# cheolwanpark/tiny-raytracer

Measured on AMD Instinct MI355X. Metric: Mray/s (primary+secondary), higher is better.
Workload: dtype f32; 1 GPU; cornell 2048x2048, depth 50, 256 spp per step (of 4096), streamed, reference-order BVH, seed 1; rays=160658711950, samples=22548578304, image_rows_per_gpu=2048, tuning=default, parallelism=single GPU, world_size=1, launched_by=plain

## Files before the change

### tiny-raytracer_amd/csrc/capi.hip

```cpp
#include <hip/hip_runtime.h>

#include <math.h>
#include <stdio.h>
#include <stdlib.h>
#include <string.h>

#include <algorithm>
#include <memory>
#include <mutex>
#include <new>
#include <string>
#include <thread>
#include <vector>

#include "axis_quads.h"
#include "nearest_first.h"
#include "flat_reuse.h"
#include "host_stage.h"
#include "kernels.h"
#include "scene.h"
#include "scene_adopt.h"
#include "scene_cache.h"
#include "scene_query.h"
#include "stream_plan.h"
// ... 29 lines not shown
        if (hipEventCreate(&ev) != hipSuccess) { (void)hipGetLastError(); return; }
        if (hipEventRecord(ev, stream) != hipSuccess) { (void)hipGetLastError(); (void)hipEventDestroy(ev); return; }
        t_open.ev = ev; t_open.stream = stream; t_open.device = dev; t_open.epoch = epoch;
        return;
    }
    if (!t_open.ev) return;
    TimingOpen o = t_open;
    t_open = TimingOpen{};
    hipEvent_t ev = nullptr;
    if (o.stream != stream || o.device != dev || o.epoch != epoch || hipEventCreate(&ev) != hipSuccess) {
        (void)hipGetLastError();
        (void)hipEventDestroy(o.ev);
        return;
    }
    if (hipEventRecord(ev, stream) != hipSuccess) { (void)hipGetLastError(); (void)hipEventDestroy(ev); (void)hipEventDestroy(o.ev); return; }
    std::lock_guard<std::mutex> lock(g_timing_mu);
    if (g_timing_on && g_timing_epoch == epoch) g_timing_pairs.push_back(TimingPair{o.ev, ev, dev});
    else { (void)hipEventDestroy(o.ev); (void)hipEventDestroy(ev); }
}
}

struct trt_scene {
    SceneHost host;
    FlatReuse flat_reuse{};
    std::vector<uint32_t> geo_index;
    SceneCache cache;
};

namespace {

thread_local std::string g_last_error;

int fail(int code, const std::string& msg) {
    g_last_error = msg;
    return code;
}
int fail_hip(hipError_t e, const char* what) {
    return fail(TRT_ERR_HIP, std::string(what) + ": " + hipGetErrorString(e));
}
#define TRT_HIP(call)                                        \
    do {                                                     \
        hipError_t e_ = (call);                              \
        if (e_ != hipSuccess) return fail_hip(e_, #call);    \
    } while (0)

struct Defaults {
    trt_tuning tuning;
    trt_scene_options scene;
    bool flat_reuse = true;
    bool axis_quads = true;
    bool nearest_first = true;
    uint32_t flat_literal = 2;
    bool flat_literal_test_fail = false;
};
const Defaults& defaults() {
    static const Defaults d = [] {
        Defaults x;
        x.tuning = tuning_builtin();
        x.scene = scene_options_builtin();
        auto env = [](const char* name) -> const char* { const char* e = getenv(name); return (e && *e) ? e : nullptr; };
        auto u32 = [&](const char* name, uint32_t& field) { if (const char* e = env(name)) field = (uint32_t)strtoul(e, nullptr, 10); };
        trt_tuning& t = x.tuning;
        u32("TRT_STREAM_MINW", t.stream_waves_per_simd); u32("TRT_BIG_THREADS", t.stream_big_threads); u32("TRT_STREAM_BATCH_SPP", t.stream_batch_spp);
        u32("TRT_RADIANCE_GB", t.radiance_gb); u32("TRT_LEAF_SLOTS", t.leaf_slots); u32("TRT_LDS_LEAF_STACK", t.lds_leaf_stack);
        u32("TRT_RAY_POOL", t.ray_pool); u32("TRT_STRAGGLERS", t.stragglers); u32("TRT_LDS_STRAGGLERS", t.lds_stragglers);
        u32("TRT_DUAL_WALK", t.dual_walk); u32("TRT_RUNTIME_WALK", t.runtime_walk); u32("TRT_XCD_REMAP", t.xcd_remap);
        u32("TRT_MINW", t.mega_waves_per_simd); u32("TRT_MEGA_THREADS", t.mega_threads); u32("TRT_MINW8", t.mega_global_waves8);
        u32("TRT_WF_MINW", t.wf_waves_per_simd); u32("TRT_WF_SERVE_MIN", t.wf_serve_min);
        trt_scene_options& o = x.scene;
        if (const char* e = env("TRT_CULL_PRUNE")) {
            const float v = (float)atof(e);
            if (v > 0.0f && v <= 1.0f) o.cull_prune = v;
        }
        if (const char* e = env("TRT_FLAT_WALK")) o.flat_walk = atoi(e) ? 1 : 0;
        if (const char* e = env("TRT_FLAT_REUSE")) x.flat_reuse = atoi(e) != 0;
        if (const char* e = env("TRT_AXIS_QUADS")) x.axis_quads = atoi(e) != 0;
        if (const char* e = env("TRT_NEAREST_FIRST")) x.nearest_first = atoi(e) != 0;
        if (const char* e = env("TRT_FLAT_LITERAL")) x.flat_literal = atoi(e) != 0 ? 1u : 0u;
        if (const char* e = env("TRT_FLAT_LITERAL_TEST_FAIL")) x.flat_literal_test_fail = atoi(e) != 0;
        if (const char* e = env("TRT_COMPACT_NODES")) o.compact_nodes = atoi(e) ? 1 : 0;
        if (const char* e = env("TRT_SCRATCH_CAP_MB")) o.scratch_cap_bytes = (uint64_t)strtoull(e, nullptr, 10) << 20;
        return x;
    }();
    return d;
}

[[maybe_unused]] const bool g_defaults_read_at_load = (defaults(), true);

int require_device() {
    int n = 0;
    hipError_t e = hipGetDeviceCount(&n);
    if (e != hipSuccess || n <= 0) {
        (void)hipGetLastError();
        return fail(TRT_ERR_NO_DEVICE, "no HIP device visible: libtinyrt has no CPU path, it needs a gfx950 GPU");
    }
    return TRT_OK;
}

int scene_on_device(trt_scene* s, SceneDev& out) {
    out.L = s->host.layout;
    return s->cache.on_device(SceneCache::PACKED_SCENE, s->host.blob.data(), s->host.layout.blob_bytes, "scene upload", out.blob);
}

void to_camera_dev(const trt_camera& c, CameraDev& d) {
    const trt_vec3* src[6] = {&c.position, &c.viewport_upper_left, &c.horizontal, &c.vertical, &c.defocus_disk_u, &c.defocus_disk_v};
    float* dst[6] = {d.pos, d.upper_left, d.horizontal, d.vertical, d.du, d.dv};
    for (int i = 0; i < 6; i++) { dst[i][0] = src[i]->x; dst[i][1] = src[i]->y; dst[i][2] = src[i]->z; }
    d.width = c.width;
    d.height = c.height;
}

int to_render_args(const trt_camera* cam, const trt_render_params* p, RenderArgs& ra, uint32_t& rows, trt_tuning& tn) {
    if (cam->width < 2 || cam->height < 2) return fail(TRT_ERR_INVALID_ARG, "camera width and height must be at least 2 (pointgen.rs:41-42 divides by width-1, height-1)");
    if (p->samples_per_pixel == 0) return fail(TRT_ERR_INVALID_ARG, "samples_per_pixel must be positive");
    uint32_t s1 = p->sample_end == 0 ? p->samples_per_pixel : p->sample_end;
    if (p->sample_begin > s1 || s1 > p->samples_per_pixel) return fail(TRT_ERR_INVALID_ARG, "sample range must satisfy begin <= end <= samples_per_pixel");
    if (p->backend > TRT_BACKEND_STREAMED) return fail(TRT_ERR_INVALID_ARG, "unknown backend");
    ra.background[0] = p->background.x; ra.background[1] = p->background.y; ra.background[2] = p->background.z;
    ra.inv_spp = 1.0f / (float)p->samples_per_pixel;
    ra.max_bounces = p->max_bounces;
    ra.seed_key = rng_seed_key(p->seed);
    ra.sample_begin = p->sample_begin;
    ra.sample_end = s1;
    ra.accumulate = p->accumulate ? 1u : 0u;
    if (p->band_rows == 0) {
        ra.band_rows = 0; ra.band_stride = 1; ra.band_offset = 0;
        rows = cam->height;
    } else {
        if (p->band_stride == 0 || p->band_offset >= p->band_stride) return fail(TRT_ERR_INVALID_ARG, "band_offset must be below band_stride");
        rows = p->rows_local;
        if (rows > 0) {
            uint32_t last = rows - 1;
// ... 39 lines not shown
    ra.flat_reuse = s->flat_reuse;
    const size_t bytes = (size_t)rows * cam->width * 3 * sizeof(float);
    if (rows == 0 || ra.sample_begin == ra.sample_end || ra.max_bounces == 0) {
        if (!ra.accumulate && bytes) TRT_HIP(hipMemsetAsync(d_accum, 0, bytes, stream));
        if (!ra.accumulate && bytes && d_moment2) TRT_HIP(hipMemsetAsync(d_moment2, 0, bytes, stream));
        return TRT_OK;
    }
    const bool wavefront = p->backend == TRT_BACKEND_WAVEFRONT;
    const bool streamed = p->backend == TRT_BACKEND_STREAMED || p->backend == TRT_BACKEND_AUTO;
    if (wavefront || streamed) {
        int dev = 0;
        TRT_HIP(hipGetDevice(&dev));
        Workspace* ws = nullptr;
        if (wavefront) {
            rc = s->cache.workspace_acquire(dev, wavefront_workspace_bytes(cam->width, rows), stream, &ws);
        } else {
            uint32_t samples = ra.sample_end - ra.sample_begin;
            const uint32_t full = streamed_chunk_spp(cam->width, rows, tn.radiance_gb);
            if (samples > full) samples = full;
            const uint32_t wanted = samples;
            const uint32_t short_samples = s->cache.short_samples(dev);
            if (short_samples != 0u && short_samples < samples) {
                const size_t idle = s->cache.idle_workspace_bytes(dev);
                size_t free_b = 0, total_b = 0;
                const bool known = hipMemGetInfo(&free_b, &total_b) == hipSuccess;
                (void)hipGetLastError();
                if (!known || free_b + idle < streamed_workspace_bytes(cam->width, rows, samples, tn.radiance_gb)) samples = short_samples;
            }
            bool trimmed = false;
            for (;;) {
                rc = s->cache.workspace_acquire(dev, streamed_workspace_bytes(cam->width, rows, samples, tn.radiance_gb), stream, &ws);
                if (rc != TRT_ERR_OOM) break;
                if (!trimmed) {
                    trimmed = true;
                    s->cache.trim(dev, 0);
                    continue;
                }
                if (samples <= 1u) break;
                samples = (samples + 1u) / 2u;
            }
            s->cache.set_short_samples(dev, (rc == TRT_OK && samples < wanted) ? samples : 0u);
        }
        if (rc != TRT_OK) return rc;
        LiteralRequest lit;
        const SceneLayout& L = s->host.layout;
        if (streamed && defaults().flat_literal != 0u && L.flat_walk != 0u && L.n_leaves > 0u &&
            s->host.blob.size() >= 16u * ((size_t)L.off_leaf_list + 2u * (size_t)L.n_leaves)) {
            lit.slot = s->cache.literal_kernel(dev);
            lit.leaf_list = s->host.blob.data() + 16u * (size_t)L.off_leaf_list;
            lit.n_leaves = L.n_leaves;
            const uint64_t call_samples = (uint64_t)cam->width * rows * (ra.sample_end - ra.sample_begin);
            lit.wanted = defaults().flat_literal == 1u || call_samples >= kLiteralAutoSamples;
            lit.empty_source = defaults().flat_literal_test_fail;
        }
        const LiteralScope lit_scope(lit.slot ? &lit : nullptr);
        hipError_t le;
        if (streamed && d_moment2) {
            le = launch_moments ? launch_moments(sc, cd, ra, tn, ws->ptr, ws->bytes, d_accum, d_moment2, reinterpret_cast<unsigned long long*>(d_counters),
                                                 p->collect_stats != 0, stream)
                                : hipErrorInvalidDeviceFunction;
        } else if (streamed) {
            le = launch_streamed(sc, cd, ra, tn, ws->ptr, ws->bytes, d_accum, reinterpret_cast<unsigned long long*>(d_counters), p->collect_stats != 0, stream);
        } else {
            le = launch_wavefront(sc, cd, ra, tn, ws->ptr, d_accum, reinterpret_cast<unsigned long long*>(d_counters), p->collect_stats != 0, stream);
        }
        rc = s->cache.workspace_release(dev, ws, stream);
        if (le != hipSuccess) return fail_hip(le, streamed ? "launch_streamed" : "launch_wavefront");
        return rc;
    }
    TRT_HIP(launch_megakernel(sc, cd, ra, tn, d_accum, reinterpret_cast<unsigned long long*>(d_counters), p->collect_stats != 0, stream));
    return TRT_OK;
}

void set_flat_reuse(trt_scene* s) {
    const SceneLayout& L = s->host.layout;
    const size_t end = 16u * ((size_t)L.off_leaf_list + 2u * (size_t)L.n_leaves);
    const bool have = L.flat_walk != 0u && L.n_leaves > 0u && s->host.blob.size() >= end;
    uint32_t m[3];
    flat_reuse_masks(have ? s->host.blob.data() + 16u * (size_t)L.off_leaf_list : nullptr, L.n_leaves, have && defaults().flat_reuse, m);
    const size_t qend = 16u * ((size_t)L.off_quad + 5u * (size_t)L.n_quads);
    const bool have_quads = have && L.n_quads > 0u && s->host.blob.size() >= qend;
    const uint32_t aq = axis_quads_flag(have_quads ? s->host.blob.data() + 16u * (size_t)L.off_quad : nullptr, L.n_quads, L.n_leaves, L.flat_walk != 0u,
                                        scene_mode(L) == 1, defaults().axis_quads);
    float planes[3];
    const uint32_t nf = nearest_first_flag(have ? s->host.blob.data() + 16u * (size_t)L.off_leaf_list : nullptr, L.n_leaves,
                                           have_quads ? s->host.blob.data() + 16u * (size_t)L.off_quad : nullptr, L.n_quads, L.n_spheres, aq,
                                           defaults().nearest_first, planes);
    s->flat_reuse = FlatReuse{m[0], m[1], m[2], aq, nf, planes[0], planes[1], planes[2]};
}

void set_geo_index(trt_scene* s) {
    const SceneLayout& L = s->host.layout;
    const std::vector<int32_t>& geo = s->host.reference.prim_geo;
    s->geo_index.assign((size_t)L.n_spheres + L.n_quads, 0xFFFFFFFFu);
    const size_t end = 16u * ((size_t)L.off_ref_nodes + 2u * (size_t)L.n_nodes);
    if (geo.size() < L.n_nodes || s->host.blob.size() < end) return;
    for (uint32_t i = 0; i < L.n_nodes; i++) {
        if (geo[i] < 0) continue;
        uint32_t link;
        memcpy(&link, s->host.blob.data() + 16u * ((size_t)L.off_ref_nodes + 2u * (size_t)i + 1u) + 12u, 4);
        const size_t slot = (size_t)(link & PRIM_INDEX_MASK) + ((link & PRIM_QUAD_BIT) ? L.n_spheres : 0u);
        if (!(link & NODE_INNER_BIT) && slot < s->geo_index.size()) s->geo_index[slot] = (uint32_t)geo[i];
    }
}

trt_scene* scene_from_host(SceneHost&& host, const trt_scene_options& opt) {
// ... 652 lines not shown
```

### tiny-raytracer_amd/csrc/flat_literal.h

```cpp
#pragma once

#include <stdint.h>
#include <stdio.h>
#include <string.h>

#include <string>

#include "flat_reuse.h"

namespace trt {

constexpr uint32_t kFlatLiteralMaxLeaves = 32u;

namespace flat_literal_detail {

inline void hex(std::string& s, uint32_t bits) {
    char b[16];
    snprintf(b, sizeof b, "0x%08x", bits);
    s += b;
}

inline void box(std::string& s, const uint32_t w[8], uint32_t axes) {
    static const char* const o[3] = {"%[ox]", "%[oy]", "%[oz]"};
    static const char* const inv[3] = {"%[ix]", "%[iy]", "%[iz]"};
// ... 31 lines not shown
inline bool flat_literal_asm(const void* leaf_list, uint32_t n_leaves, const uint32_t masks[3], std::string& out) {
    using namespace flat_literal_detail;
    if (leaf_list == nullptr || n_leaves == 0u || n_leaves > kFlatLiteralMaxLeaves) return false;
    const unsigned char* p = static_cast<const unsigned char*>(leaf_list);
    const uint32_t n = n_leaves;
    auto leaf = [&](uint32_t k, uint32_t w[8]) { memcpy(w, p + 32u * (size_t)k, 32u); };
    auto axes_of = [&](uint32_t k) {
        const uint32_t b = 1u << k;
        return k == 0u ? 7u : (((masks[0] & b) ? 0u : 1u) | ((masks[1] & b) ? 0u : 2u) | ((masks[2] & b) ? 0u : 4u));
    };
    std::string s;
    uint32_t w[8];
    s += "s_cmp_lg_u32 %[i], 0\n";
    s += "s_cbranch_scc1 900f\n";
    for (uint32_t k = 0; k < n; k++) {
        label(s, 200u, k);
        leaf(k, w);
        box(s, w, axes_of(k));
        if ((k & 1u) && k + 1u < n) {
            s += "v_cmp_gt_u32_e32 vcc, %[top], %[lim]\n";
            s += "s_cbranch_vccnz "; ref(s, 400u, k + 1u, 'f'); s += "\n";
        }
    }
    s += "s_mov_b32 %[i], "; hex(s, n); s += "\n";
    s += "s_branch 990f\n";
    for (uint32_t k = 2; k < n; k += 2u) {
        label(s, 400u, k);
        s += "s_mov_b32 %[i], "; hex(s, k); s += "\n";
        s += "s_branch 990f\n";
    }
    for (uint32_t k = 2; k < n; k += 2u) {
        if (axes_of(k) == 7u) continue;
        label(s, 100u, k);
        leaf(k, w);
        box(s, w, 7u);
        if (k + 1u < n) { s += "s_branch "; ref(s, 200u, k + 1u, 'b'); s += "\n"; }
        else { s += "s_mov_b32 %[i], "; hex(s, n); s += "\n"; s += "s_branch 990f\n"; }
    }
    s += "900:\n";
    s += "s_lshl_b32 s38, %[i], 1\n";
    s += "s_add_u32 s38, s38, 12\n";
    s += "s_getpc_b64 s[36:37]\n";
    s += "s_add_u32 s36, s36, s38\n";
    s += "s_addc_u32 s37, s37, 0\n";
    s += "s_setpc_b64 s[36:37]\n";
    for (uint32_t k = 0; k < n; k += 2u) {
        s += "s_branch "; ref(s, axes_of(k) == 7u ? 200u : 100u, k, 'b'); s += "\n";
    }
    s += "990:\n";
    out.swap(s);
    return true;
}

inline std::string flat_literal_define(const std::string& name, const std::string& asm_text) {
    std::string d = "#define " + name + " \\\n";
    size_t a = 0;
    while (a < asm_text.size()) {
        size_t b = asm_text.find('\n', a);
        if (b == std::string::npos) b = asm_text.size();
        d += "\""; d.append(asm_text, a, b - a); d += "\\n\" \\\n";
        a = b + 1u;
    }
    d += "\"\"\n";
    return d;
}

}
```

### tiny-raytracer_amd/csrc/flat_literal_rtc.h

```cpp
#pragma once

#include <dlfcn.h>
#include <stdint.h>

#include <string>
#include <vector>

#include "flat_literal.h"

namespace trt {

struct RtcHeader { const char* name; const char* text; };
inline const std::vector<RtcHeader>& rtc_project_headers() {
    static const std::vector<RtcHeader> h = {
#include "rtc_headers.inc"
    };
    return h;
}
inline const std::vector<RtcHeader>& rtc_system_headers() {
    static const std::vector<RtcHeader> h = {
        {"hip/hip_runtime.h", "#pragma once\n"},
        {"stdint.h", "#pragma once\n"
                     "typedef signed char int8_t; typedef unsigned char uint8_t; typedef short int16_t; typedef unsigned short uint16_t;\n"
                     "typedef int int32_t; typedef unsigned int uint32_t; typedef long int64_t; typedef unsigned long uint64_t;\n"
                     "typedef unsigned long uintptr_t; typedef long intptr_t;\n"},
        {"stddef.h", "#pragma once\n#ifndef offsetof\n#define offsetof(t, m) __builtin_offsetof(t, m)\n#endif\n"},
        {"string.h", "#pragma once\ninline void* memcpy(void* d, const void* s, unsigned long n) { return __builtin_memcpy(d, s, n); }\n"},
        {"math.h", "#pragma once\n"},
    };
    return h;
}

struct HiprtcApi {
    typedef void* Program;
    int (*create)(Program*, const char*, const char*, int, const char* const*, const char* const*) = nullptr;
    int (*destroy)(Program*) = nullptr;
    int (*add_name)(Program, const char*) = nullptr;
    int (*compile)(Program, int, const char* const*) = nullptr;
    int (*log_size)(Program, size_t*) = nullptr;
    int (*log)(Program, char*) = nullptr;
    int (*lowered)(Program, const char*, const char**) = nullptr;
    int (*code_size)(Program, size_t*) = nullptr;
    int (*code)(Program, char*) = nullptr;
    bool ok = false;
};
inline const HiprtcApi& hiprtc_api(const void* beside) {
    static const HiprtcApi api = [beside] {
        HiprtcApi a;
        void* h = nullptr;
        for (const char* name : {"libhiprtc.so", "libhiprtc.so.7", "libhiprtc.so.6"}) {
            h = dlopen(name, RTLD_NOW | RTLD_LOCAL);
            if (h) break;
        }
        Dl_info info;
        if (!h && beside && dladdr(beside, &info) && info.dli_fname) {
            std::string dir(info.dli_fname);
            const size_t slash = dir.rfind('/');
            if (slash != std::string::npos) h = dlopen((dir.substr(0, slash + 1) + "libhiprtc.so").c_str(), RTLD_NOW | RTLD_LOCAL);
        }
        if (!h) return a;
        auto sym = [&](auto& fn, const char* name) { fn = reinterpret_cast<std::remove_reference_t<decltype(fn)>>(dlsym(h, name)); return fn != nullptr; };
        a.ok = sym(a.create, "hiprtcCreateProgram") && sym(a.destroy, "hiprtcDestroyProgram") && sym(a.add_name, "hiprtcAddNameExpression") &&
               sym(a.compile, "hiprtcCompileProgram") && sym(a.log_size, "hiprtcGetProgramLogSize") && sym(a.log, "hiprtcGetProgramLog") &&
               sym(a.lowered, "hiprtcGetLoweredName") && sym(a.code_size, "hiprtcGetCodeSize") && sym(a.code, "hiprtcGetCode");
        return a;
    }();
    return api;
}

struct FlatLiteralBuild {
    std::vector<char> code;
    std::string kernel;
    std::string log;
};

inline std::string flat_literal_source(const std::string& asm_text) {
    return flat_literal_define("TRT_FLAT_LITERAL_ASM", asm_text) + "#include \"stream_pool.h\"\n";
}

inline bool flat_literal_compile(const std::string& source, int minw, const char* arch, const void* beside, FlatLiteralBuild& out) {
    const HiprtcApi& rtc = hiprtc_api(beside);
    if (!rtc.ok) { out.log = "hiprtc not found"; return false; }
    std::vector<const char*> names, texts;
    for (const auto* set : {&rtc_system_headers(), &rtc_project_headers()})
        for (const RtcHeader& h : *set) { names.push_back(h.name); texts.push_back(h.text); }
    HiprtcApi::Program prog = nullptr;
    if (rtc.create(&prog, source.c_str(), "stream_pool_literal.hip", (int)names.size(), texts.data(), names.data()) != 0) { out.log = "hiprtcCreateProgram failed"; return false; }
    const std::string expr = "&trt::stream_pool_kernel<1, false, " + std::to_string(minw) + ", 256, 2, true>";
    const std::string arch_opt = std::string("--offload-arch=") + arch;
    const char* opts[] = {arch_opt.c_str(), "-O3", "-std=c++17", "-ffp-contract=off", "-fno-fast-math", "-fno-slp-vectorize"};
    int rc = rtc.add_name(prog, expr.c_str());
    if (rc == 0) rc = rtc.compile(prog, (int)(sizeof(opts) / sizeof(opts[0])), opts);
    size_t n = 0;
    if (rtc.log_size(prog, &n) == 0 && n > 1) { out.log.resize(n); rtc.log(prog, &out.log[0]); }
    bool ok = rc == 0;
    const char* lowered = nullptr;
    if (ok) ok = rtc.lowered(prog, expr.c_str(), &lowered) == 0 && lowered != nullptr;
    if (ok) out.kernel = lowered;
    if (ok) ok = rtc.code_size(prog, &n) == 0 && n > 0;
    if (ok) { out.code.resize(n); ok = rtc.code(prog, out.code.data()) == 0; }
    if (!ok && out.log.empty()) out.log = "hiprtc failed (" + std::to_string(rc) + ")";
    rtc.destroy(&prog);
    return ok;
}

}
```

### tiny-raytracer_amd/csrc/literal_kernel.h

```cpp
#pragma once

#include <stdint.h>

#include <condition_variable>
#include <mutex>

namespace trt {

struct LiteralKernel {
    enum State { UNTRIED, COMPILING, READY, FAILED };
    std::mutex mu;
    std::condition_variable cv;
    State state = UNTRIED;
    void* module = nullptr;
    void* function = nullptr;
    int minw = 0;
    void (*unload)(void* module) = nullptr;
    void release() {
        if (module && unload) unload(module);
        module = function = nullptr;
        state = UNTRIED;
    }
};

struct LiteralRequest {
    LiteralKernel* slot = nullptr;
    const void* leaf_list = nullptr;
    uint32_t n_leaves = 0;
    bool wanted = false;
    bool empty_source = false;
};
inline thread_local const LiteralRequest* t_literal_request = nullptr;
class LiteralScope {
  public:
    explicit LiteralScope(const LiteralRequest* r) { t_literal_request = r; }
    LiteralScope(const LiteralScope&) = delete;
    ~LiteralScope() { t_literal_request = nullptr; }
};

constexpr uint64_t kLiteralAutoSamples = 1ull << 26;

}
```

### tiny-raytracer_amd/csrc/rt_path.h

```cpp
#pragma once

#include "axis_quads.h"
#include "nearest_first.h"
#include "kernels.h"
#include "rt_device.h"
#include "stream_plan.h"

namespace trt {

extern __shared__ float4 g_lds[];


template <int MODE>
struct SceneAcc {
    const float4* blob;
    SceneLayout L;
    TRT_DEV float4 f4(uint32_t idx) const { return MODE == MODE_LDS ? g_lds[idx] : blob[idx]; }
    TRT_DEV uint32_t u32(uint32_t idx) const {
        return MODE == MODE_LDS ? reinterpret_cast<const uint32_t*>(g_lds)[idx] : reinterpret_cast<const uint32_t*>(blob)[idx];
    }
    TRT_DEV void node(uint32_t i, float4& a, float4& b) const { a = f4(2u * i); b = f4(2u * i + 1u); }
    TRT_DEV void ref_node(uint32_t i, float4& a, float4& b) const { a = blob[L.off_ref_nodes + 2u * i]; b = blob[L.off_ref_nodes + 2u * i + 1u]; }
    TRT_DEV float4 sphere(uint32_t i) const { return f4(L.off_sphere + i); }
    TRT_DEV float4 quad(uint32_t plane, uint32_t i) const { return f4(L.off_quad + 5u * i + plane); }
// ... 409 lines not shown
    "v_sub_f32_e32 %[t0], " LOZ ", %[oz]\n v_sub_f32_e32 %[t1], " HIZ ", %[oz]\n v_mul_f32_e32 %[t0], %[iz], %[t0]\n"                  \
    "v_mul_f32_e32 %[t1], %[iz], %[t1]\n v_min_f32_e32 %[ze], %[t0], %[t1]\n v_max_f32_e32 %[zx], %[t0], %[t1]\n"                        \
    "12:\n v_max3_f32 %[st], %[xe], %[ye], %[ze]\n v_min3_f32 %[t0], %[xx], %[yx], %[zx]\n v_cmp_nle_f32_e32 vcc, %[t0], %[st]\n"

TRT_DEV float2* box_loop_flat(const Trav& tr, const V3& o, const float4* __restrict__ leaf_list, uint32_t& i, uint32_t n, float2* stk, float2* limit,
                              FlatReuse reuse) {
    const uint32_t stk_off = lds_offset(stk);
    uint32_t top = stk_off;
    const uint32_t lim = lds_offset(limit);
    const uint32_t first = ~(1u << (i & 31u));
    const uint32_t rx = reuse.x & first, ry = reuse.y & first, rz = reuse.z & first;
    unsigned long long m;
    uint32_t off;
    float t0, t1, xe, xx, ye, yx, ze, zx, st, lk;
    asm volatile(
        "s_lshl_b32 %[off], %[i], 5\n"
        "s_load_dwordx16 s[36:51], %[list], %[off]\n"
        "1:\n"
        "s_waitcnt lgkmcnt(0)\n"
        TRT_FLAT_BOX("s36", "s37", "s38", "s39", "s40", "s41")
        "s_and_saveexec_b64 %[m], vcc\n"
        "v_mov_b32_e32 %[lk], s43\n"
        "ds_write2_b32 %[top], %[lk], %[st] offset1:1\n"
        "v_add_u32_e32 %[top], 0x200, %[top]\n"
        "s_mov_b64 exec, %[m]\n"
        "s_add_u32 %[i], %[i], 1\n"
        "s_cmp_ge_u32 %[i], %[n]\n"
        "s_cbranch_scc1 2f\n"
        TRT_FLAT_BOX("s44", "s45", "s46", "s47", "s48", "s49")
        "v_mov_b32_e32 %[lk], s51\n"
        "s_add_u32 %[off], %[off], 64\n"
        "s_load_dwordx16 s[36:51], %[list], %[off]\n"
        "s_and_saveexec_b64 %[m], vcc\n"
        "ds_write2_b32 %[top], %[lk], %[st] offset1:1\n"
        "v_add_u32_e32 %[top], 0x200, %[top]\n"
        "s_mov_b64 exec, %[m]\n"
        "s_add_u32 %[i], %[i], 1\n"
        "v_cmp_gt_u32_e32 vcc, %[top], %[lim]\n"
        "s_cmp_lg_u64 vcc, 0\n"
        "s_cbranch_scc1 2f\n"
        "s_cmp_lt_u32 %[i], %[n]\n"
        "s_cbranch_scc1 1b\n"
        "2:\n"
        "s_waitcnt lgkmcnt(0)\n"
        : [i] "+s"(i), [top] "+v"(top), [m] "=&s"(m), [off] "=&s"(off), [t0] "=&v"(t0), [t1] "=&v"(t1), [xe] "=&v"(xe), [xx] "=&v"(xx),
          [ye] "=&v"(ye), [yx] "=&v"(yx), [ze] "=&v"(ze), [zx] "=&v"(zx), [st] "=&v"(st), [lk] "=&v"(lk)
        : [n] "s"(n), [list] "s"(leaf_list), [lim] "v"(lim), [ox] "v"(o.x), [oy] "v"(o.y), [oz] "v"(o.z), [ix] "v"(tr.inv.x), [iy] "v"(tr.inv.y),
          [iz] "v"(tr.inv.z), [tb] "v"(tr.t_best), [tmin] "s"(kTMin), [rx] "s"(rx), [ry] "s"(ry), [rz] "s"(rz)
        : "vcc", "scc", "memory", "s36", "s37", "s38", "s39", "s40", "s41", "s42", "s43", "s44", "s45", "s46", "s47", "s48", "s49", "s50", "s51");
    return stk + ((top - stk_off) >> 3);
}

#ifdef TRT_FLAT_LITERAL_ASM
TRT_DEV float2* box_loop_flat_literal(const Trav& tr, const V3& o, uint32_t& i, float2* stk, float2* limit) {
    const uint32_t stk_off = lds_offset(stk);
    uint32_t top = stk_off;
    const uint32_t lim = lds_offset(limit);
    unsigned long long m;
    float t0, t1, xe, xx, ye, yx, ze, zx, st, lk;
    asm volatile(
        TRT_FLAT_LITERAL_ASM
        : [i] "+s"(i), [top] "+v"(top), [m] "=&s"(m), [t0] "=&v"(t0), [t1] "=&v"(t1), [xe] "=&v"(xe), [xx] "=&v"(xx),
          [ye] "=&v"(ye), [yx] "=&v"(yx), [ze] "=&v"(ze), [zx] "=&v"(zx), [st] "=&v"(st), [lk] "=&v"(lk)
        : [lim] "v"(lim), [ox] "v"(o.x), [oy] "v"(o.y), [oz] "v"(o.z), [ix] "v"(tr.inv.x), [iy] "v"(tr.inv.y),
          [iz] "v"(tr.inv.z), [tb] "v"(tr.t_best), [tmin] "s"(kTMin)
        : "vcc", "scc", "memory", "s36", "s37", "s38");
    return stk + ((top - stk_off) >> 3);
}
#endif

struct FlatIntervals {
    float xe, xx, ye, yx, ze, zx;
};
TRT_DEV bool flat_box(FlatIntervals& c, float4 na, float4 nb, V3 o, V3 inv, uint32_t axes, float start, float end, float& start_out) {
    if (axes & 1u) { const float x0 = (na.x - o.x) * inv.x, x1 = (na.w - o.x) * inv.x; c.xe = __builtin_fminf(x0, x1); c.xx = __builtin_fmaxf(x0, x1); }
    if (axes & 2u) { const float y0 = (na.y - o.y) * inv.y, y1 = (nb.x - o.y) * inv.y; c.ye = __builtin_fminf(y0, y1); c.yx = __builtin_fmaxf(y0, y1); }
    if (axes & 4u) { const float z0 = (na.z - o.z) * inv.z, z1 = (nb.y - o.z) * inv.z; c.ze = __builtin_fminf(z0, z1); c.zx = __builtin_fmaxf(z0, z1); }
    const float tn = __builtin_fmaxf(__builtin_fmaxf(c.xe, c.ye), c.ze);
    const float tf = __builtin_fminf(__builtin_fminf(c.xx, c.yx), c.zx);
    start = __builtin_fmaxf(start, tn);
    end = __builtin_fminf(end, tf);
    start_out = start;
    return !(end <= start);
}
TRT_DEV uint32_t flat_axes(const FlatReuse& r, uint32_t i) {
    const uint32_t b = 1u << (i & 31u);
    return ((r.x & b) ? 0u : 1u) | ((r.y & b) ? 0u : 2u) | ((r.z & b) ? 0u : 4u);
}

template <int MODE, bool STATS, bool ANY = false>
TRT_DEV void walk_flat(const SceneAcc<MODE>& sc, const float4* __restrict__ leaf_list, const Ray& ray, Trav& tr, Counters<STATS>& ctr,
                       float2* stk, uint32_t slots, FlatReuse reuse) {
    const uint32_t n = sc.L.n_leaves;
    uint32_t i = 0;
    const bool nearest = !STATS && !ANY && reuse.nearest_first != 0u;
    const float margin = nearest ? nf_margin(reuse.px, reuse.py, reuse.pz, ray.o.x, ray.o.y, ray.o.z, tr.inv.x, tr.inv.y, tr.inv.z) : 0.0f;
    auto phase = [&](const float2* top) {
        if constexpr (!STATS && !ANY) {
            if (nearest) { leaf_phase_nearest<MODE>(sc, ray, stk, top, tr, margin); return; }
        }
        leaf_phase<MODE, STATS>(stk, top, tr, ctr, [&](uint32_t leaf) { trav_leaf<MODE, STATS, !STATS>(sc, ray, tr, leaf, ctr, reuse.axis_quads); });
    };
    if constexpr (kAsmBoxLoop && !STATS) {
        float2* const lim = stk + 64u * (slots - 2u);
        do {
#ifdef TRT_FLAT_LITERAL_ASM
            float2* const top = box_loop_flat_literal(tr, ray.o, i, stk, lim);
#else
            float2* const top = box_loop_flat(tr, ray.o, leaf_list, i, n, stk, lim, reuse);
#endif
            TRT_CLK(ctr, 1);
            phase(top);
            TRT_CLK(ctr, 2);
            if constexpr (ANY) { if (__builtin_amdgcn_ballot_w64(tr.prim_best == PRIM_NONE) == 0ull) return; }
        } while (i < n);
        return;
// ... 495 lines not shown
```

### tiny-raytracer_amd/csrc/streamed.hip

```cpp
#include <mutex>
#include <string>

#include "flat_literal_rtc.h"
#include "host_stage.h"
#include "kernels.h"
#include "literal_kernel.h"
#include "rt_path.h"
#include "stream_plan.h"
#include "stream_pool.h"
#include "wave_run.h"

namespace trt {

template <int MODE, bool STATS, int MINW = 1, int THREADS = 256, int WALK = WALK_RUNTIME, bool LAZY = false>
__global__ __launch_bounds__(THREADS, MINW) void stream_sample_kernel(SceneDev scd, CameraDev cam, RenderArgs ra,
                                                                             float* __restrict__ colors,
                                                                             uint32_t* __restrict__ batch_counter,
                                                                             unsigned long long* __restrict__ counters,
                                                                             uint32_t tiles_x, uint32_t n_tiles, uint32_t n_batches, uint32_t batch_spp,
                                                                             const float4* __restrict__ leaf_list,
                                                                             const uint4* __restrict__ nodes16) {
    stage_scene_to_lds<MODE>(scd);
    const FlatReuse flat_reuse = axis_quads_to_lds<MODE, STATS, WALK>(scd, ra.flat_reuse);
    const SceneAcc<MODE> sc{scd.blob, scd.L};
// ... 297 lines not shown
    return c;
}
constexpr size_t kWorkspaceHeader = 256;
size_t streamed_workspace_bytes(uint32_t width, uint32_t rows, uint32_t samples, uint32_t radiance_gb) {
    const uint32_t chunk = streamed_chunk_spp(width, rows, radiance_gb);
    return kWorkspaceHeader + (size_t)padded_pixels(width, rows) * (samples < chunk ? (samples ? samples : 1u) : chunk) * 3 * sizeof(float);
}
uint32_t streamed_chunk_that_fits(uint32_t width, uint32_t rows, size_t bytes) {
    const unsigned long long px = padded_pixels(width, rows);
    if (px == 0 || bytes <= kWorkspaceHeader) return 0;
    unsigned long long c = (bytes - kWorkspaceHeader) / (px * 12ull);
    if (c > 256ull) c = 256ull;
    while (c > 1ull && px * c >= (1ull << 32)) c--;
    return (uint32_t)c;
}

namespace {

#define TRT_FN_POOL(MODE, STATS, MINW, THREADS, WALK, LAZY) reinterpret_cast<const void*>(&stream_pool_kernel<MODE, STATS, MINW, THREADS, WALK, LAZY>),
#define TRT_FN_SAMPLE(MODE, STATS, MINW, THREADS, WALK, LAZY) reinterpret_cast<const void*>(&stream_sample_kernel<MODE, STATS, MINW, THREADS, WALK, LAZY>),
#define TRT_FN_DUAL(MINW) reinterpret_cast<const void*>(&stream_dual_kernel<MINW, 256>),
const void* const kStreamKernelFns[] = {
    TRT_STREAM_SPECIALISED(TRT_FN_POOL, TRT_FN_SAMPLE, TRT_FN_DUAL)
    TRT_STREAM_GENERAL(TRT_FN_POOL, TRT_FN_SAMPLE, TRT_FN_DUAL)
};
#undef TRT_FN_POOL
#undef TRT_FN_SAMPLE
#undef TRT_FN_DUAL
static_assert(sizeof(kStreamKernelFns) / sizeof(kStreamKernelFns[0]) == kStreamKernelCount, "one address per shape row");

std::mutex g_literal_mu;
unsigned long long g_literal_compilations = 0;
std::string g_literal_diagnostic;
thread_local std::string t_literal_diagnostic_copy;

void literal_unload(void* module) {
    (void)hipModuleUnload(static_cast<hipModule_t>(module));
    (void)hipGetLastError();
}

bool literal_build(LiteralKernel& slot, const LiteralRequest& rq, const FlatReuse& reuse, int minw, std::string& why) {
    {
        std::lock_guard<std::mutex> lock(g_literal_mu);
        g_literal_compilations++;
    }
    int dev = 0;
    hipDeviceProp_t prop;
    if (hipGetDevice(&dev) != hipSuccess || hipGetDeviceProperties(&prop, dev) != hipSuccess) { (void)hipGetLastError(); why = "no device properties"; return false; }
    std::string arch(prop.gcnArchName);
    arch = arch.substr(0, arch.find(':'));
    const uint32_t masks[3] = {reuse.x, reuse.y, reuse.z};
    std::string text, source;
    if (!rq.empty_source) {
        if (!flat_literal_asm(rq.leaf_list, rq.n_leaves, masks, text)) { why = "leaf list refused"; return false; }
        source = flat_literal_source(text);
    }
    FlatLiteralBuild built;
    if (!flat_literal_compile(source, minw, arch.c_str(), reinterpret_cast<const void*>(&hipModuleLoadData), built)) { why = "hiprtc: " + built.log; return false; }
    hipModule_t mod = nullptr;
    hipFunction_t fn = nullptr;
    hipError_t e = hipModuleLoadData(&mod, built.code.data());
    if (e == hipSuccess) e = hipModuleGetFunction(&fn, mod, built.kernel.c_str());
    if (e != hipSuccess) {
        (void)hipGetLastError();
        if (mod) (void)hipModuleUnload(mod);
        why = std::string("module load: ") + hipGetErrorString(e);
        return false;
    }
    slot.module = mod; slot.function = fn; slot.minw = minw; slot.unload = &literal_unload;
    return true;
}

hipFunction_t literal_kernel_for(const StreamLaunchPlan& pl, const RenderArgs& ra, bool stats) {
    const LiteralRequest* rq = t_literal_request;
#ifdef TRT_PHASE_CLOCK
    return nullptr;
#endif
    if (!kAsmBoxLoop) return nullptr;
    if (!rq || !rq->slot || stats || !pl.specialised || !pl.pool || pl.dual || pl.walk != WALK_FLAT || pl.mode != MODE_LDS || ra.ref_tree ||
        pl.kernel_walk != WALK_FLAT || pl.threads != 256 || pl.lds_bytes > 48u * 1024u || rq->n_leaves > kFlatLiteralMaxLeaves) return nullptr;
    LiteralKernel& slot = *rq->slot;
    std::unique_lock<std::mutex> lock(slot.mu);
    while (slot.state == LiteralKernel::COMPILING) slot.cv.wait(lock);
    if (slot.state == LiteralKernel::UNTRIED && rq->wanted) {
        slot.state = LiteralKernel::COMPILING;
        lock.unlock();
        std::string why;
        const bool ok = literal_build(slot, *rq, ra.flat_reuse, pl.kernel_minw, why);
        if (!ok) {
            std::lock_guard<std::mutex> g(g_literal_mu);
            g_literal_diagnostic = "lock-step kernel not compiled for its scene, the built-in kernel runs: " + why;
        }
        lock.lock();
        slot.state = ok ? LiteralKernel::READY : LiteralKernel::FAILED;
        slot.cv.notify_all();
    }
    if (slot.state != LiteralKernel::READY || slot.minw != pl.kernel_minw) return nullptr;
    return static_cast<hipFunction_t>(slot.function);
}

}

static hipError_t launch_streamed_folds(const SceneDev& sc, const CameraDev& cam, const RenderArgs& ra_all, const trt_tuning& tn, void* workspace, size_t workspace_bytes,
                                        float* d_accum, float* d_moment2, unsigned long long* d_counters, bool stats, hipStream_t stream) {
    if (ra_all.rows_local == 0 || cam.width == 0) return hipSuccess;
    uint32_t* batch_counter = static_cast<uint32_t*>(workspace);
    float* colors = reinterpret_cast<float*>(static_cast<char*>(workspace) + kWorkspaceHeader);
    const uint32_t samples_all = ra_all.sample_end - ra_all.sample_begin;
// ... 133 lines not shown
```

Baseline: 71420 Mray/s.

## Cache slab intervals and plane distances in registers for the literal flat-leaf walk

The runtime-generated assembly for the flat leaf-box loop gains a register-allocation pass. Identical per-axis slab intervals across leaves are kept in extra VGPR pairs, and repeated plane constants keep their (plane - origin) * inv distances in dedicated registers, with evictions chosen by furthest next use. This is meant to remove redundant sub/mul/min/max work per ray when many leaves share walls, as in the Cornell scene. The cost is up to 18 extra VGPR outputs in the inline asm, which can raise register pressure and lower occupancy; the original loop stays as a fallback path.

Measured after the change: 78480 Mray/s (median of 6 runs). 1.1x the previous value.

```diff
diff --git a/tiny-raytracer_amd/csrc/capi.hip b/tiny-raytracer_amd/csrc/capi.hip
--- a/tiny-raytracer_amd/csrc/capi.hip
+++ b/tiny-raytracer_amd/csrc/capi.hip
@@ -105,6 +105,8 @@
     bool nearest_first = true;
     uint32_t flat_literal = 2;
     bool flat_literal_test_fail = false;
+    uint32_t flat_literal_pairs = kLiteralIntervalPairs;
+    uint32_t flat_literal_planes = kLiteralPlaneRegs;
 };
 const Defaults& defaults() {
     static const Defaults d = [] {
@@ -131,6 +133,8 @@
         if (const char* e = env("TRT_NEAREST_FIRST")) x.nearest_first = atoi(e) != 0;
         if (const char* e = env("TRT_FLAT_LITERAL")) x.flat_literal = atoi(e) != 0 ? 1u : 0u;
         if (const char* e = env("TRT_FLAT_LITERAL_TEST_FAIL")) x.flat_literal_test_fail = atoi(e) != 0;
+        if (const char* e = env("TRT_FLAT_LITERAL_PAIRS")) { const int v = atoi(e); if (v >= 3 && v <= 8) x.flat_literal_pairs = (uint32_t)v; }
+        if (const char* e = env("TRT_FLAT_LITERAL_PLANES")) { const int v = atoi(e); if (v >= 0 && v <= 8 && *e >= '0' && *e <= '9') x.flat_literal_planes = (uint32_t)v; }
         if (const char* e = env("TRT_COMPACT_NODES")) o.compact_nodes = atoi(e) ? 1 : 0;
         if (const char* e = env("TRT_SCRATCH_CAP_MB")) o.scratch_cap_bytes = (uint64_t)strtoull(e, nullptr, 10) << 20;
         return x;
@@ -276,6 +280,8 @@
             const uint64_t call_samples = (uint64_t)cam->width * rows * (ra.sample_end - ra.sample_begin);
             lit.wanted = defaults().flat_literal == 1u || call_samples >= kLiteralAutoSamples;
             lit.empty_source = defaults().flat_literal_test_fail;
+            lit.interval_pairs = defaults().flat_reuse ? defaults().flat_literal_pairs : 3u;
+            lit.plane_regs = defaults().flat_reuse ? defaults().flat_literal_planes : 0u;
         }
         const LiteralScope lit_scope(lit.slot ? &lit : nullptr);
         hipError_t le;
diff --git a/tiny-raytracer_amd/csrc/flat_literal.h b/tiny-raytracer_amd/csrc/flat_literal.h
--- a/tiny-raytracer_amd/csrc/flat_literal.h
+++ b/tiny-raytracer_amd/csrc/flat_literal.h
@@ -107,6 +107,169 @@
     return true;
 }
 
+struct FlatCacheStats {
+    uint32_t intervals = 0;
+    uint32_t plane_distances = 0;
+    uint32_t evictions = 0;
+    uint32_t far_reuses = 0;
+    uint32_t extra_operands = 0;
+    bool cached = false;
+};
+constexpr uint32_t kFlatCacheMinPairs = 3u, kFlatCacheMaxPairs = 8u, kFlatCacheMaxPlanes = 8u;
+constexpr uint32_t kFlatCacheMaxExtra = 2u * (kFlatCacheMaxPairs - 3u) + kFlatCacheMaxPlanes;
+
+inline bool flat_literal_cached_asm(const void* leaf_list, uint32_t n_leaves, const uint32_t masks[3], uint32_t interval_pairs, uint32_t plane_regs,
+                                    std::string& out, FlatCacheStats& stats) {
+    using namespace flat_literal_detail;
+    if (interval_pairs < kFlatCacheMinPairs || interval_pairs > kFlatCacheMaxPairs || plane_regs > kFlatCacheMaxPlanes) return false;
+    std::string plain;
+    if (!flat_literal_asm(leaf_list, n_leaves, masks, plain)) return false;
+    const unsigned char* p = static_cast<const unsigned char*>(leaf_list);
+    const uint32_t n = n_leaves, kNever = 0xffffffffu;
+    uint32_t w[kFlatLiteralMaxLeaves][8];
+    for (uint32_t k = 0; k < n; k++) memcpy(w[k], p + 32u * (size_t)k, 32u);
+    auto finite = [](uint32_t b) { return (b & 0x7f800000u) != 0x7f800000u; };
+    auto shareable = [&](uint32_t k, int a) { return finite(w[k][a]) && finite(w[k][3 + a]); };
+    auto same = [&](uint32_t k, uint32_t j, int a) { return w[k][a] == w[j][a] && w[k][3 + a] == w[j][3 + a]; };
+    FlatCacheStats st;
+    uint32_t plain_intervals = 0;
+    for (uint32_t k = 0; k < n; k++)
+        for (int a = 0; a < 3; a++) plain_intervals += (k == 0u || !(masks[a] & (1u << k))) ? 1u : 0u;
+    struct Pair { bool used = false; int axis = 0; uint32_t leaf = 0; bool share = false; };
+    Pair pairs[kFlatCacheMaxPairs];
+    uint32_t slot_of[kFlatLiteralMaxLeaves][3];
+    bool computed[kFlatLiteralMaxLeaves][3];
+    auto next_use = [&](const Pair& q, uint32_t after) {
+        if (!q.used || !q.share) return kNever;
+        for (uint32_t j = after + 1u; j < n; j++) if (shareable(j, q.axis) && same(j, q.leaf, q.axis)) return 3u * j + (uint32_t)q.axis;
+        return kNever;
+    };
+    for (uint32_t k = 0; k < n; k++) {
+        bool needed[kFlatCacheMaxPairs] = {};
+        uint32_t found[3] = {kNever, kNever, kNever};
+        for (int a = 0; a < 3; a++) {
+            if (!shareable(k, a)) continue;
+            for (uint32_t s = 0; s < interval_pairs; s++)
+                if (pairs[s].used && pairs[s].share && pairs[s].axis == a && same(k, pairs[s].leaf, a)) { found[a] = s; needed[s] = true; break; }
+        }
+        for (int a = 0; a < 3; a++) {
+            if (found[a] != kNever) {
+                slot_of[k][a] = found[a]; computed[k][a] = false;
+                if (k == 0u || !(masks[a] & (1u << k))) st.far_reuses++;
+                continue;
+            }
+            uint32_t best = kNever, best_use = 0;
+            for (uint32_t s = 0; s < interval_pairs; s++) {
+                if (needed[s]) continue;
+                const uint32_t u = next_use(pairs[s], k);
+                if (best == kNever || u > best_use) { best = s; best_use = u; }
+            }
+            if (best_use != kNever) st.evictions++;
+            pairs[best] = Pair{true, a, k, shareable(k, a)};
+            needed[best] = true;
+            slot_of[k][a] = best; computed[k][a] = true;
+            st.intervals++;
+        }
+    }
+    struct Use { uint32_t leaf; int axis; int hi; uint32_t bits; bool share; };
+    Use uses[6u * kFlatLiteralMaxLeaves];
+    uint32_t n_uses = 0;
+    for (uint32_t k = 0; k < n; k++)
+        for (int a = 0; a < 3; a++)
+            if (computed[k][a])
+                for (int h = 0; h < 2; h++) { const uint32_t b = w[k][3 * h + a]; uses[n_uses++] = Use{k, a, h, b, finite(b)}; }
+    auto plane_next = [&](int axis, uint32_t bits, uint32_t after) {
+        for (uint32_t j = after + 1u; j < n_uses; j++) if (uses[j].share && uses[j].axis == axis && uses[j].bits == bits) return j;
+        return kNever;
+    };
+    struct Plane { bool used = false; int axis = 0; uint32_t bits = 0; };
+    Plane planes[kFlatCacheMaxPlanes];
+    uint32_t reg_of[6u * kFlatLiteralMaxLeaves];
+    bool written[6u * kFlatLiteralMaxLeaves];
+    for (uint32_t u = 0; u < n_uses; u++) {
+        reg_of[u] = kNever; written[u] = true;
+        if (!uses[u].share || plane_regs == 0u) { st.plane_distances++; continue; }
+        uint32_t hit = kNever;
+        for (uint32_t r = 0; r < plane_regs; r++) if (planes[r].used && planes[r].axis == uses[u].axis && planes[r].bits == uses[u].bits) { hit = r; break; }
+        if (hit != kNever) { reg_of[u] = hit; written[u] = false; continue; }
+        st.plane_distances++;
+        const uint32_t mine = plane_next(uses[u].axis, uses[u].bits, u);
+        if (mine == kNever) continue;
+        const uint32_t partner = uses[u].hi ? reg_of[u - 1u] : kNever;
+        uint32_t best = kNever, best_use = 0;
+        for (uint32_t r = 0; r < plane_regs; r++) {
+            if (r == partner) continue;
+            const uint32_t v = planes[r].used ? plane_next(planes[r].axis, planes[r].bits, u) : kNever;
+            if (best == kNever || v > best_use) { best = r; best_use = v; }
+        }
+        if (best == kNever || best_use <= mine) continue;
+        planes[best] = Plane{true, uses[u].axis, uses[u].bits};
+        reg_of[u] = best;
+    }
+    const bool gains = st.intervals < plain_intervals || st.plane_distances < 2u * plain_intervals;
+    if ((interval_pairs == kFlatCacheMinPairs && plane_regs == 0u) || !gains) {
+        stats = FlatCacheStats{};
+        stats.intervals = plain_intervals; stats.plane_distances = 2u * plain_intervals;
+        out.swap(plain);
+        return true;
+    }
+    static const char* const o[3] = {"%[ox]", "%[oy]", "%[oz]"};
+    static const char* const inv[3] = {"%[ix]", "%[iy]", "%[iz]"};
+    static const char* const first_lo[3] = {"%[xe]", "%[ye]", "%[ze]"};
+    static const char* const first_hi[3] = {"%[xx]", "%[yx]", "%[zx]"};
+    auto c = [](uint32_t j) { return "%[c" + std::to_string(j) + "]"; };
+    auto pair_lo = [&](uint32_t s) { return s < 3u ? std::string(first_lo[s]) : c(2u * (s - 3u)); };
+    auto pair_hi = [&](uint32_t s) { return s < 3u ? std::string(first_hi[s]) : c(2u * (s - 3u) + 1u); };
+    auto plane_reg = [&](uint32_t r) { return c(2u * (interval_pairs - 3u) + r); };
+    std::string s;
+    s += "s_cmp_lg_u32 %[i], 0\n";
+    s += "s_cbranch_scc1 1000f\n";
+    uint32_t u = 0;
+    for (uint32_t k = 0; k < n; k++) {
+        label(s, 1200u, k);
+        for (int a = 0; a < 3; a++) {
+            if (!computed[k][a]) continue;
+            std::string d[2];
+            for (int h = 0; h < 2; h++) {
+                d[h] = reg_of[u + h] != kNever ? plane_reg(reg_of[u + h]) : (h ? "%[t1]" : "%[t0]");
+                if (written[u + h]) { s += "v_sub_f32_e32 " + d[h] + ", "; hex(s, uses[u + h].bits); s += ", "; s += o[a]; s += "\n"; }
+            }
+            for (int h = 0; h < 2; h++)
+                if (written[u + h]) { s += "v_mul_f32_e32 " + d[h] + ", "; s += inv[a]; s += ", " + d[h] + "\n"; }
+            const std::string lo = pair_lo(slot_of[k][a]), hi = pair_hi(slot_of[k][a]);
+            if (a == 0) {
+                s += "v_med3_f32 " + lo + ", " + d[0] + ", " + d[1] + ", %[tmin]\n";
+                s += "v_med3_f32 " + hi + ", " + d[0] + ", " + d[1] + ", %[tb]\n";
+            } else {
+                s += "v_min_f32_e32 " + lo + ", " + d[0] + ", " + d[1] + "\n";
+                s += "v_max_f32_e32 " + hi + ", " + d[0] + ", " + d[1] + "\n";
+            }
+            u += 2u;
+        }
+        s += "v_max3_f32 %[st], " + pair_lo(slot_of[k][0]) + ", " + pair_lo(slot_of[k][1]) + ", " + pair_lo(slot_of[k][2]) + "\n";
+        s += "v_min3_f32 %[t0], " + pair_hi(slot_of[k][0]) + ", " + pair_hi(slot_of[k][1]) + ", " + pair_hi(slot_of[k][2]) + "\n";
+        s += "v_cmp_nle_f32_e32 vcc, %[t0], %[st]\n";
+        s += "s_and_saveexec_b64 %[m], vcc\n";
+        s += "v_mov_b32_e32 %[lk], "; hex(s, w[k][7]); s += "\n";
+        s += "ds_write2_b32 %[top], %[lk], %[st] offset1:1\n";
+        s += "v_add_u32_e32 %[top], 0x200, %[top]\n";
+        s += "s_mov_b64 exec, %[m]\n";
+        if ((k & 1u) && k + 1u < n) {
+            s += "v_cmp_gt_u32_e32 vcc, %[top], %[lim]\n";
+            s += "s_cbranch_vccnz "; ref(s, 400u, k + 1u, 'f'); s += "\n";
+        }
+    }
+    s += "s_mov_b32 %[i], "; hex(s, n); s += "\n";
+    s += "s_branch 990f\n";
+    s += "1000:\n";
+    s += plain;
+    st.extra_operands = 2u * (interval_pairs - 3u) + plane_regs;
+    st.cached = true;
+    stats = st;
+    out.swap(s);
+    return true;
+}
+
 inline std::string flat_literal_define(const std::string& name, const std::string& asm_text) {
     std::string d = "#define " + name + " \\\n";
     size_t a = 0;
diff --git a/tiny-raytracer_amd/csrc/flat_literal_rtc.h b/tiny-raytracer_amd/csrc/flat_literal_rtc.h
--- a/tiny-raytracer_amd/csrc/flat_literal_rtc.h
+++ b/tiny-raytracer_amd/csrc/flat_literal_rtc.h
@@ -74,8 +74,9 @@
     std::string log;
 };
 
-inline std::string flat_literal_source(const std::string& asm_text) {
-    return flat_literal_define("TRT_FLAT_LITERAL_ASM", asm_text) + "#include \"stream_pool.h\"\n";
+inline std::string flat_literal_source(const std::string& asm_text, uint32_t extra_operands = 0u) {
+    return flat_literal_define("TRT_FLAT_LITERAL_ASM", asm_text) + "#define TRT_FLAT_LITERAL_EXTRA " + std::to_string(extra_operands) +
+           "\n#include \"stream_pool.h\"\n";
 }
 
 inline bool flat_literal_compile(const std::string& source, int minw, const char* arch, const void* beside, FlatLiteralBuild& out) {
diff --git a/tiny-raytracer_amd/csrc/literal_kernel.h b/tiny-raytracer_amd/csrc/literal_kernel.h
--- a/tiny-raytracer_amd/csrc/literal_kernel.h
+++ b/tiny-raytracer_amd/csrc/literal_kernel.h
@@ -23,12 +23,16 @@
     }
 };
 
+constexpr uint32_t kLiteralIntervalPairs = 8u, kLiteralPlaneRegs = 6u;
+
 struct LiteralRequest {
     LiteralKernel* slot = nullptr;
     const void* leaf_list = nullptr;
     uint32_t n_leaves = 0;
     bool wanted = false;
     bool empty_source = false;
+    uint32_t interval_pairs = kLiteralIntervalPairs;
+    uint32_t plane_regs = kLiteralPlaneRegs;
 };
 inline thread_local const LiteralRequest* t_literal_request = nullptr;
 class LiteralScope {
diff --git a/tiny-raytracer_amd/csrc/rt_path.h b/tiny-raytracer_amd/csrc/rt_path.h
--- a/tiny-raytracer_amd/csrc/rt_path.h
+++ b/tiny-raytracer_amd/csrc/rt_path.h
@@ -485,16 +485,42 @@
 }
 
 #ifdef TRT_FLAT_LITERAL_ASM
+#ifndef TRT_FLAT_LITERAL_EXTRA
+#define TRT_FLAT_LITERAL_EXTRA 0
+#endif
+#define TRT_FLC_0
+#define TRT_FLC_1 TRT_FLC_0, [c0] "=&v"(c[0])
+#define TRT_FLC_2 TRT_FLC_1, [c1] "=&v"(c[1])
+#define TRT_FLC_3 TRT_FLC_2, [c2] "=&v"(c[2])
+#define TRT_FLC_4 TRT_FLC_3, [c3] "=&v"(c[3])
+#define TRT_FLC_5 TRT_FLC_4, [c4] "=&v"(c[4])
+#define TRT_FLC_6 TRT_FLC_5, [c5] "=&v"(c[5])
+#define TRT_FLC_7 TRT_FLC_6, [c6] "=&v"(c[6])
+#define TRT_FLC_8 TRT_FLC_7, [c7] "=&v"(c[7])
+#define TRT_FLC_9 TRT_FLC_8, [c8] "=&v"(c[8])
+#define TRT_FLC_10 TRT_FLC_9, [c9] "=&v"(c[9])
+#define TRT_FLC_11 TRT_FLC_10, [c10] "=&v"(c[10])
+#define TRT_FLC_12 TRT_FLC_11, [c11] "=&v"(c[11])
+#define TRT_FLC_13 TRT_FLC_12, [c12] "=&v"(c[12])
+#define TRT_FLC_14 TRT_FLC_13, [c13] "=&v"(c[13])
+#define TRT_FLC_15 TRT_FLC_14, [c14] "=&v"(c[14])
+#define TRT_FLC_16 TRT_FLC_15, [c15] "=&v"(c[15])
+#define TRT_FLC_17 TRT_FLC_16, [c16] "=&v"(c[16])
+#define TRT_FLC_18 TRT_FLC_17, [c17] "=&v"(c[17])
+#define TRT_FLC_CAT2(a, b) a##b
+#define TRT_FLC_CAT(a, b) TRT_FLC_CAT2(a, b)
 TRT_DEV float2* box_loop_flat_literal(const Trav& tr, const V3& o, uint32_t& i, float2* stk, float2* limit) {
     const uint32_t stk_off = lds_offset(stk);
     uint32_t top = stk_off;
     const uint32_t lim = lds_offset(limit);
     unsigned long long m;
     float t0, t1, xe, xx, ye, yx, ze, zx, st, lk;
+    [[maybe_unused]] float c[18];
     asm volatile(
         TRT_FLAT_LITERAL_ASM
         : [i] "+s"(i), [top] "+v"(top), [m] "=&s"(m), [t0] "=&v"(t0), [t1] "=&v"(t1), [xe] "=&v"(xe), [xx] "=&v"(xx),
           [ye] "=&v"(ye), [yx] "=&v"(yx), [ze] "=&v"(ze), [zx] "=&v"(zx), [st] "=&v"(st), [lk] "=&v"(lk)
+          TRT_FLC_CAT(TRT_FLC_, TRT_FLAT_LITERAL_EXTRA)
         : [lim] "v"(lim), [ox] "v"(o.x), [oy] "v"(o.y), [oz] "v"(o.z), [ix] "v"(tr.inv.x), [iy] "v"(tr.inv.y),
           [iz] "v"(tr.inv.z), [tb] "v"(tr.t_best), [tmin] "s"(kTMin)
         : "vcc", "scc", "memory", "s36", "s37", "s38");
diff --git a/tiny-raytracer_amd/csrc/streamed.hip b/tiny-raytracer_amd/csrc/streamed.hip
--- a/tiny-raytracer_amd/csrc/streamed.hip
+++ b/tiny-raytracer_amd/csrc/streamed.hip
@@ -373,8 +373,9 @@
     const uint32_t masks[3] = {reuse.x, reuse.y, reuse.z};
     std::string text, source;
     if (!rq.empty_source) {
-        if (!flat_literal_asm(rq.leaf_list, rq.n_leaves, masks, text)) { why = "leaf list refused"; return false; }
-        source = flat_literal_source(text);
+        FlatCacheStats cache;
+        if (!flat_literal_cached_asm(rq.leaf_list, rq.n_leaves, masks, rq.interval_pairs, rq.plane_regs, text, cache)) { why = "leaf list refused"; return false; }
+        source = flat_literal_source(text, cache.extra_operands);
     }
     FlatLiteralBuild built;
     if (!flat_literal_compile(source, minw, arch.c_str(), reinterpret_cast<const void*>(&hipModuleLoadData), built)) { why = "hiprtc: " + built.log; return false; }
```
